# MitchellHansen/voxel-raycaster

Measured on AMD Instinct MI355X. Metric: Mrays/s (primary+shadow), 1920x1080 into depth-12 SVO, higher is better.
Workload: dtype f32

## Files before the change

### __graft_entry__.py

```python
import os
import subprocess
import sys

ROOT = os.path.dirname(os.path.abspath(__file__))
PKG = os.path.join(ROOT, "voxel-raycaster_amd")
CSRC = os.path.join(PKG, "csrc")
HIPCC = os.environ.get("HIPCC", "/opt/rocm/bin/hipcc")
HIP_FLAGS = ["--offload-arch=gfx950", "-O3", "-std=c++17", "-ffp-contract=off", "-fno-slp-vectorize", "-fPIC",
             "-I" + os.path.join(ROOT, "include")]
SOURCES = ["raycast_kernel.hip", "raycast_jump_kernel.hip", "svo_builder_gpu.hip", "empty_boxes.hip", "raycast_query.hip", "box_query.hip", "box_sweep.hip",
           "vrc_api.cpp", "svo_builder.cpp"]
HEADERS = ["vrc_params.h", "raycast_common.hpp", "exact_jump.hpp", "safe_run.hpp", "clcaster.hpp", "shell_scene.hpp", "raycast_query.h",
           "box_query.h", "box_walk.hpp", "box_sweep.h", "vrc_launch.h"]


def _stale(target, deps):
    if not os.path.exists(target):
        return True
    t = os.path.getmtime(target)
    return any(os.path.getmtime(d) > t for d in deps)


def stale() -> bool:
    srcs = [os.path.join(CSRC, s) for s in SOURCES]
    hdrs = [os.path.join(CSRC, h) for h in HEADERS] + [os.path.join(ROOT, "include", "vrc.h")]
    orc = os.path.join(ROOT, "oracle")
    return (_stale(os.path.join(PKG, "libvrc.so"), srcs + hdrs)
            or _stale(os.path.join(orc, "libvrc_oracle.so"), [os.path.join(orc, "vrc_oracle.c"), os.path.join(orc, "vrc_oracle.h")]))
# ... 79 lines not shown
```

### include/vrc.h

```cpp
#ifndef VRC_H
#define VRC_H

#include <stddef.h>
#include <stdint.h>

#ifdef __cplusplus
extern "C" {
#endif

typedef struct vrc_caster vrc_caster;

typedef enum vrc_status {
    VRC_OK = 0,
    VRC_ERR_INVALID_ARGUMENT = 1,
    VRC_ERR_NOT_READY = 2,
    VRC_ERR_DEVICE = 3,
    VRC_ERR_OUT_OF_MEMORY = 4,
    VRC_ERR_NOT_FOUND = 5,
    VRC_ERR_LIMIT = 6
} vrc_status;


int vrc_create(int device_ordinal, vrc_caster **out);
int vrc_destroy(vrc_caster *h);
// ... 134 lines not shown
#define VRC_KERNEL_SVO   1
#define VRC_KERNEL_JUMP  2
#define VRC_KERNEL_ARRAY 3
typedef struct vrc_kernel_info {
    uint32_t struct_size;
    int32_t  family;
    int32_t  n_args;
    int32_t  args[6];
    int32_t  jump_min_run;
    int32_t  lds_rows;
    int32_t  reserved_;
    char     name[96];
} vrc_kernel_info;
int vrc_last_kernel(vrc_caster *h, int32_t rank, vrc_kernel_info *out);

int vrc_get_scheduler_stats(vrc_caster *h, uint64_t out[8]);

int vrc_timing_reset(vrc_caster *h);
int vrc_timing_get(vrc_caster *h, uint64_t *n_launches, double *total_kernel_ms);


int vrc_octree_generate(const int8_t *grid, uint32_t dim, uint64_t buffer_size,
                        int strict_reference, uint64_t **descriptors,
                        uint64_t *n_descriptors, uint64_t *root_index);

int vrc_octree_attachments_from_grid(const int8_t *grid, uint32_t dim, const uint64_t *descriptors,
                                     uint64_t n_descriptors, uint64_t root_index, uint32_t **lookup,
                                     uint64_t **attachments, uint64_t *n_attachments);
int vrc_scene_shell_terrain_attachments(uint32_t depth, uint64_t seed, uint32_t mirror_period,
                                        const uint64_t *descriptors, uint64_t n_descriptors,
// ... 63 lines not shown
```

### voxel-raycaster_amd/__init__.py

```python
from __future__ import annotations

import ctypes as C
import os
from typing import Optional

import numpy as np

_HERE = os.path.dirname(os.path.abspath(__file__))
LIB_PATH = os.environ.get("VRC_LIB_PATH") or os.path.join(_HERE, "libvrc.so")


class VrcError(RuntimeError):
    pass


def _load() -> C.CDLL:
    try:
        import torch
    except ImportError:
        pass
    if not os.path.exists(LIB_PATH):
        raise VrcError(
            f"{LIB_PATH} is missing: build it with `python -c 'import __graft_entry__ as g; g.build()'` "
            "(hipcc --offload-arch=gfx950).  There is no CPU fallback.")
# ... 77 lines not shown
    "vrc_setting_set": (C.c_int, [_H, C.c_char_p, C.c_int64]),
    "vrc_setting_get": (C.c_int, [_H, C.c_char_p, C.POINTER(C.c_int64)]),
    "vrc_validate": (C.c_int, [_H]),
    "vrc_prepare": (C.c_int, [_H]),
    "vrc_compute": (C.c_int, [_H]),
    "vrc_compute_async": (C.c_int, [_H]),
    "vrc_sync": (C.c_int, [_H]),
    "vrc_set_row_tiling": (C.c_int, [_H, C.c_int32, C.c_int32, C.c_int32]),
    "vrc_read_image_f32": (C.c_int, [_H, _f32p, C.c_size_t]),
    "vrc_read_image_rgba8": (C.c_int, [_H, _u8p, C.c_size_t]),
    "vrc_read_hits": (C.c_int, [_H, _i32p, C.c_size_t]),
    "vrc_device_image": (C.c_int, [_H, C.POINTER(C.c_void_p), C.POINTER(C.c_size_t)]),
    "vrc_get_counters": (C.c_int, [_H, C.POINTER(Counters)]),
    "vrc_counters_canonical": (C.c_int, [_H, C.POINTER(C.c_int32)]),
    "vrc_last_kernel": (C.c_int, [_H, C.c_int32, C.POINTER(KernelInfo)]),
    "vrc_get_scheduler_stats": (C.c_int, [_H, _u64p]),
    "vrc_timing_reset": (C.c_int, [_H]),
    "vrc_timing_get": (C.c_int, [_H, _u64p, C.POINTER(C.c_double)]),
    "vrc_octree_generate": (C.c_int, [_i8p, C.c_uint32, C.c_uint64, C.c_int, C.POINTER(_u64p), _u64p, _u64p]),
    "vrc_scene_shell_terrain": (C.c_int, [C.c_uint32, C.c_uint64, C.c_int32, C.c_int, C.POINTER(_u64p), _u64p, _u64p, _i32p]),
    "vrc_octree_attachments_from_grid": (C.c_int, [_i8p, C.c_uint32, _u64p, C.c_uint64, C.c_uint64,
                                                    C.POINTER(C.POINTER(C.c_uint32)), C.POINTER(_u64p), _u64p]),
    "vrc_scene_shell_terrain_attachments": (C.c_int, [C.c_uint32, C.c_uint64, C.c_uint32, _u64p, C.c_uint64, C.c_uint64,
                                                       C.POINTER(C.POINTER(C.c_uint32)), C.POINTER(_u64p), _u64p]),
    "vrc_scene_shell_terrain_dense": (C.c_int, [C.c_uint32, C.c_uint64, C.c_int32, _i8p]),
    "vrc_scene_atlas": (C.c_int, [C.c_int32, C.c_int32, _u8p]),
    "vrc_octree_get_voxel": (C.c_int, [_u64p, C.c_uint64, C.c_uint32, _i32p, _i32p, _i32p, _i32p]),
    "vrc_octree_save": (C.c_int, [C.c_char_p, C.c_uint32, _u64p, C.c_uint64, C.c_uint64, C.POINTER(C.c_uint32), _u64p, C.c_uint64]),
    "vrc_octree_load": (C.c_int, [C.c_char_p, C.POINTER(C.c_uint32), C.POINTER(_u64p), _u64p, _u64p,
                                  C.POINTER(C.POINTER(C.c_uint32)), C.POINTER(_u64p), _u64p]),
# ... 580 lines not shown
    def sweep_boxes_device(self, sweeps_ptr: int, n: int, records_ptr: int, max_events: int = 0, stopping_only: bool = False) -> bool:
        return self._ok(lib.vrc_sweep_boxes_device(self._h, C.c_void_p(sweeps_ptr), int(n), int(max_events),
                                                   SWEEP_STOPPING_ONLY if stopping_only else 0, C.c_void_p(records_ptr)))

    def counters(self) -> dict:
        c = Counters()
        if not self._ok(lib.vrc_get_counters(self._h, C.byref(c))):
            raise VrcError(self.last_error())
        d = c.as_dict()
        canonical = C.c_int32(-1)
        if lib.vrc_counters_canonical(self._h, C.byref(canonical)) != 0:
            raise RuntimeError(self.last_error())
        d["canonical_reads"] = bool(canonical.value)
        return d

    def last_kernel(self, rank: int = 0) -> dict:
        k = KernelInfo()
        k.struct_size = C.sizeof(KernelInfo)
        if not self._ok(lib.vrc_last_kernel(self._h, rank, C.byref(k))):
            raise VrcError(self.last_error())
        return {"family": int(k.family), "args": tuple(int(a) for a in k.args[:k.n_args]), "name": k.name.decode(),
                "jump_min_run": int(k.jump_min_run), "lds_rows": int(k.lds_rows)}

    def scheduler_stats(self) -> dict:
        out = (C.c_uint64 * 8)()
        if not self._ok(lib.vrc_get_scheduler_stats(self._h, out)):
            raise VrcError(self.last_error())
        names = ("wave_step_iterations", "bursts", "event_passes", "event_lanes", "shade_passes", "shade_lanes", "jump_attempts", "jump_successes")
        return {n: int(out[i]) for i, n in enumerate(names)}

# ... 10 lines not shown
```

### voxel-raycaster_amd/csrc/raycast_common.hpp

```cpp
#pragma once

#include <hip/hip_runtime.h>

#include "vrc_params.h"

namespace vrc {

__device__ __forceinline__ float min_cl(float a, float b) { return b < a ? b : a; }
__device__ __forceinline__ float max_cl(float a, float b) { return a < b ? b : a; }
__device__ __forceinline__ float mix_cl(float x, float y, float a) { return x + (y - x) * a; }
__device__ __forceinline__ int isign(float v) { return (v > 0.0f) - (v < 0.0f); }
__device__ __forceinline__ float dot3(float ax, float ay, float az, float bx, float by, float bz) {
    return ax * bx + ay * by + az * bz;
}

struct Vec3 { float x, y, z; };
constexpr unsigned kCountTex = 1u, kCountShadow = 0x100u, kCountBounce = 0x10000u;

__device__ __forceinline__ Vec3 normalize3(Vec3 v) {
    float l2 = dot3(v.x, v.y, v.z, v.x, v.y, v.z);
    if (l2 == 0.0f) return v;
    float l = sqrtf(l2);
    return Vec3{v.x / l, v.y / l, v.z / l};
}
// ... 271 lines not shown
        const int w = blockIdx.x;
        bid = (w / (8 * S)) * 8 + (w & 7);
        sub = (w >> 3) % S;
    }
    return bid < nblocks;
}
template <int kTiles>
__device__ __forceinline__ bool workgroup_exists(const RaycastParams &p) {
    int nblocks, bid, sub;
    return workgroup_group<kTiles>(p, nblocks, bid, sub);
}
template <int kTiles = kTilesPerBlock>
__device__ __forceinline__ bool block_pixel(const RaycastParams &p, int &px, int &py, int &buffer_row) {
    int nblocks, bid, sub;
    if (!workgroup_group<kTiles>(p, nblocks, bid, sub)) return false;
    const int per_xcd = nblocks >> 3;
    int local_ty, bx;
    if (p.xcd_mode == 1 && per_xcd > 0 && bid < (per_xcd << 3) && (p.local_tile_rows & 7) == 0) {
        const int j = bid >> 3;
        local_ty = (j / p.blocks_x) * 8 + (bid & 7);
        bx = j % p.blocks_x;
    } else {
        if (p.xcd_mode == 0 && per_xcd > 0 && bid < (per_xcd << 3)) bid = (bid & 7) * per_xcd + (bid >> 3);
        local_ty = bid / p.blocks_x;
        bx = bid - local_ty * p.blocks_x;
    }
    const int band = local_ty / p.band_tiles;
    const int tile_y = (band * p.tile_world + p.tile_rank) * p.band_tiles + (local_ty - band * p.band_tiles);
    const int wave = sub * kTiles + (threadIdx.x >> 6), lane = threadIdx.x & 63;
    px = (bx * kTilesPerBlock + wave) * kTileW + (lane & (kTileW - 1));
// ... 50 lines not shown
```

### voxel-raycaster_amd/csrc/raycast_kernel.hip

```cpp
#include <hip/hip_runtime.h>

#include <mutex>

#include "exact_jump.hpp"
#include "raycast_common.hpp"
#include "safe_run.hpp"
#include "vrc_launch.h"

#ifndef VRC_RELIGHT_THRESHOLD
#define VRC_RELIGHT_THRESHOLD 64
#endif

namespace vrc {

static_assert(3 * 4 * (int)(sizeof(JumpWord) / sizeof(uint32_t)) == kJumpTableDwordsPerLane, "vrc_api.cpp sizes the global Euclid tables (4 ring rows x 3 pairs x 8 bytes) with kJumpTableDwordsPerLane");

__device__ __forceinline__ uint64_t make_entry(const uint64_t *__restrict__ descriptors, uint64_t index,
                                               uint64_t d) {
    uint64_t base = index + (d & 0x7fffULL);
    if (d & 0x8000ULL) base = descriptors[base];
    return (base << 16) | ((d >> 16) & 0xffffULL);
}

__global__ __launch_bounds__(kBlockThreads) void raycast_array_kernel(const RaycastParams p) {
// ... 45 lines not shown
        ray_finish(r, p, c_desc);
    }
    const unsigned vals[7] = {c_primary, c_shadow, c_desc, c_tex, c_map, c_steps, c_unwritten};
    publish_counters(p, block_ctr, vals, (int)threadIdx.x);
}

#ifndef VRC_MIN_BLOCKS
#define VRC_MIN_BLOCKS (24 / VRC_TILES_PER_BLOCK)
#endif
enum LaneMode { kStep = 0, kEvent = 1, kShade = 2, kDone = 3, kRelight = 4 };

#ifdef VRC_SCHED_STATS
__device__ unsigned long long g_run_hist[3][32];
__device__ unsigned long long g_jump_stats[12];
#endif
#ifdef VRC_TIME_STATS
__device__ unsigned long long g_time_stats[16];
#define VRC_TICK(slot) do { const unsigned long long now_ = __builtin_amdgcn_s_memtime(); if ((tid & 63) == 0) t_acc[slot] += now_ - t_last; t_last = now_; } while (0)
#else
#define VRC_TICK(slot) do { } while (0)
#endif

#ifndef VRC_MIN_BLOCKS_JUMP
#define VRC_MIN_BLOCKS_JUMP (VRC_MIN_BLOCKS - 1)
#endif
constexpr int kHwRegXccId = (3 << 11) | (0 << 6) | 20;
#ifndef VRC_MIN_BLOCKS_JUMP_MULTI
#define VRC_MIN_BLOCKS_JUMP_MULTI VRC_MIN_BLOCKS_JUMP
#endif
constexpr int svo_waves_per_simd(bool jump, bool multi) { return jump ? (multi ? VRC_MIN_BLOCKS_JUMP_MULTI : VRC_MIN_BLOCKS_JUMP) : VRC_MIN_BLOCKS; }
// ... 13 lines not shown
    const int tid = threadIdx.x;
    const int wave_in_block = __builtin_amdgcn_readfirstlane(tid >> 6);
    if (!workgroup_exists<kWgTiles>(p)) {
        if (tid < kCtrCount) p.counters[(long)blockIdx.x * kCtrCount + tid] = 0;
        return;
    }
#ifdef VRC_SCHED_STATS
    constexpr bool kCtrLds = true;
#else
    constexpr bool kCtrLds = kWgTiles > 1;
#endif
    if constexpr (kCtrLds) { if (tid < kCtrCount) block_ctr[tid] = 0; }
#ifdef VRC_TIME_STATS
    __shared__ unsigned long long s_life[3];
    if (tid < 3) s_life[tid] = 0;
#endif
    if (kJump && !kLdsTab && tid == 0) {
        const unsigned per = (unsigned)p.jump_slot_count >> 3;
        const unsigned xcc = (unsigned)__builtin_amdgcn_s_getreg(kHwRegXccId) & 7u;
        const unsigned lo = xcc * per, hi = lo + per;
        unsigned i = lo + (unsigned)(((unsigned long long)(blockIdx.x >> 3) * 2654435761ULL) % per), tries = 0;
        while (atomicCAS(&p.jump_slots[i], 0u, 1u) != 0u) {
            if (++i == hi) i = lo;
            if (++tries >= per) { i = 0xffffffffu; break; }
        }
        s_jump_slot = (int)i;
    }
    __syncthreads();

    int px, py, brow;
// ... 567 lines not shown
    if (l_ok) atomicAdd(&block_ctr[kCtrShadeLanes + 2], (unsigned long long)l_ok);
    if (l_cov) atomicAdd(&block_ctr[kCtrMap], (unsigned long long)l_cov);
#endif
#ifdef VRC_TIME_STATS
    {
        const unsigned long long now_ = __builtin_amdgcn_s_memtime();
        if ((tid_end & 63) == 0) {
            t_acc[8] = now_ - t_begin;
            for (int k = 0; k < 9; k++) atomicAdd(&g_time_stats[k], t_acc[k]);
            atomicAdd(&s_life[0], t_acc[8]);
            atomicMax(&s_life[1], t_acc[8]);
        }
        if (__ballot(c_shadow != 0) != 0 && (tid_end & 63) == 0) atomicOr(&s_life[2], 1ULL);
    }
#endif
    const unsigned vals[7] = {c_primary, c_shadow, c_desc, c_tex, 0u, c_steps, c_unwritten};
    publish_counters<kWgTiles, kCtrLds>(p, block_ctr, vals, tid_end, rounds_left < 0);
    if (kJump && !kLdsTab && tid_end == 0 && s_jump_slot >= 0) atomicExch(&p.jump_slots[s_jump_slot], 0u);
#ifdef VRC_TIME_STATS
    if constexpr (kWgTiles == 1) __syncthreads();
    if (tid_end == 0) {
        const int cls = s_life[2] ? 12 : 9;
        atomicAdd(&g_time_stats[cls], s_life[0]);
        atomicAdd(&g_time_stats[cls + 1], s_life[1] * (unsigned long long)kWgTiles);
        atomicAdd(&g_time_stats[cls + 2], 1ULL);
    }
#endif
}

__global__ void reduce_counters_kernel(const unsigned long long *partials, int nblocks, unsigned long long *out) {
    __shared__ unsigned long long acc[kCtrCount];
    if (threadIdx.x < kCtrCount) acc[threadIdx.x] = 0;
    __syncthreads();
    const int slot = threadIdx.x & (kCtrCount - 1);
    unsigned long long v = 0;
    for (int b = threadIdx.x / kCtrCount; b < nblocks; b += blockDim.x / kCtrCount) v += partials[(long)b * kCtrCount + slot];
    atomicAdd(&acc[slot], v);
    __syncthreads();
    if (threadIdx.x < kCtrCount) out[threadIdx.x] = acc[threadIdx.x];
}

__global__ void frame_setup_kernel(const RaycastParams p) {
    if (threadIdx.x != 0 || blockIdx.x != 0) return;
    int pos[3], corner[3] = {0, 0, 0};
    for (int a = 0; a < 3; a++) pos[a] = (int)floorf(p.cam_pos[a]);
    uint64_t index = p.root_index, d = p.descriptors[index];
    int reads = 1;
    int dimension = 1 << p.log2_dim, res = dimension / 2;
    while (dimension > 1) {
        const int half = dimension / 2;
        int i = 0;
        for (int a = 0; a < 3; a++)
            if (pos[a] >= corner[a] + half) { i |= 1 << a; corner[a] += half; }
        if (!((d >> (16 + i)) & 1ULL)) break;
        if ((d >> (24 + i)) & 1ULL) break;
        dimension = half;
        res /= 2;
        const int before = __popcll((d >> 16) & ((2ULL << i) - 1ULL)) - 1;
        const uint64_t base = (d & 0x8000ULL) ? p.descriptors[index + (d & 0x7fffULL)] : index + (d & 0x7fffULL);
        index = base + (uint64_t)before;
        d = p.descriptors[index];
        reads++;
    }
    for (int a = 0; a < 3; a++) p.frame[a] = p.octree_bias ? (corner[a] - pos[a]) * res / 2 : 0;
    p.frame[3] = reads;
}

__global__ void fill_image_kernel(float4 *image, size_t n) {
    const size_t i = (size_t)blockIdx.x * blockDim.x + threadIdx.x;
    if (i < n) image[i] = make_float4(1.0f, 1.0f, 1.0f, 100.0f / 255.0f);
}

__global__ void pack_rgba8_kernel(const float4 *__restrict__ image, uchar4 *__restrict__ out, size_t n) {
    const size_t i = (size_t)blockIdx.x * blockDim.x + threadIdx.x;
    if (i >= n) return;
    const float4 v = image[i];
    auto q = [](float f) -> unsigned char {
        if (!(f > 0.0f)) f = 0.0f;
        if (f > 1.0f) f = 1.0f;
        return (unsigned char)__float2int_rn(f * 255.0f);
    };
    out[i] = make_uchar4(q(v.x), q(v.y), q(v.z), q(v.w));
}

#ifdef VRC_TIME_STATS
}
extern "C" int vrc_stats_time(unsigned long long *out16, int clear) {
    if (out16 && hipMemcpyFromSymbol(out16, HIP_SYMBOL(vrc::g_time_stats), sizeof(vrc::g_time_stats)) != hipSuccess) return 1;
    if (clear) {
        static unsigned long long zero[16];
        if (hipMemcpyToSymbol(HIP_SYMBOL(vrc::g_time_stats), zero, sizeof(zero)) != hipSuccess) return 1;
    }
    return 0;
}
namespace vrc {
#endif
#ifdef VRC_SCHED_STATS
}
extern "C" int vrc_stats_run_hist(unsigned long long *out96, int clear) {
    if (out96 && hipMemcpyFromSymbol(out96, HIP_SYMBOL(vrc::g_run_hist), sizeof(vrc::g_run_hist)) != hipSuccess) return 1;
    if (out96 && hipMemcpyFromSymbol(out96 + 96, HIP_SYMBOL(vrc::g_jump_stats), sizeof(vrc::g_jump_stats)) != hipSuccess) return 1;
    if (out96 && hipMemcpyFromSymbol(out96 + 108, HIP_SYMBOL(vrc::g_jump_private_solves), sizeof(vrc::g_jump_private_solves)) != hipSuccess) return 1;
    if (clear) {
        static unsigned long long zero[3][32];
        if (hipMemcpyToSymbol(HIP_SYMBOL(vrc::g_run_hist), zero, sizeof(zero)) != hipSuccess) return 1;
        if (hipMemcpyToSymbol(HIP_SYMBOL(vrc::g_jump_stats), zero, sizeof(vrc::g_jump_stats)) != hipSuccess) return 1;
        if (hipMemcpyToSymbol(HIP_SYMBOL(vrc::g_jump_private_solves), zero, sizeof(vrc::g_jump_private_solves)) != hipSuccess) return 1;
    }
    return 0;
}
namespace vrc {
// ... 2 lines not shown
hipError_t launch_fill_image(float *image, size_t n_pixels, hipStream_t stream) {
    (void)hipGetLastError();
    if (!n_pixels) return hipSuccess;
    hipLaunchKernelGGL(fill_image_kernel, dim3((unsigned)((n_pixels + 255) / 256)), dim3(256), 0, stream, reinterpret_cast<float4 *>(image), n_pixels);
    return hipGetLastError();
}

hipError_t launch_pack_rgba8(const float *image, uint8_t *out, size_t n_pixels, hipStream_t stream) {
    (void)hipGetLastError();
    if (!n_pixels) return hipSuccess;
    hipLaunchKernelGGL(pack_rgba8_kernel, dim3((unsigned)((n_pixels + 255) / 256)), dim3(256), 0, stream,
                       reinterpret_cast<const float4 *>(image), reinterpret_cast<uchar4 *>(out), n_pixels);
    return hipGetLastError();
}

hipError_t launch_frame_setup(const RaycastParams &p, hipStream_t stream) {
    (void)hipGetLastError();
    hipLaunchKernelGGL(frame_setup_kernel, dim3(1), dim3(64), 0, stream, p);
    return hipGetLastError();
}

static bool svo_uses_coarse(const RaycastParams &p) {
    return p.coarse != nullptr && p.coarse_log2 >= 1 && p.coarse_log2 <= p.log2_dim - 2;
}
static bool svo_uses_boxes(const RaycastParams &p) { return svo_uses_coarse(p) && p.boxes != nullptr && p.box_aux != nullptr; }
static bool svo_jumps(const RaycastParams &p) { return p.jump_min_run < kJumpOff; }
static int svo_tiles(bool jump, bool multi) { return svo_tiles_per_workgroup(jump, multi); }
static size_t svo_stack_bytes(const RaycastParams &p, int tiles) {
    const int levels = svo_uses_coarse(p) ? p.log2_dim - p.coarse_log2 : (p.log2_dim > 1 ? p.log2_dim - 1 : 1);
    return (size_t)levels * 64 * tiles * (sizeof(uint64_t) + (svo_uses_boxes(p) ? sizeof(uint32_t) : 0)) + (size_t)p.lds_pad_bytes * tiles / kTilesPerBlock;
}
constexpr size_t lds_table_bytes(int rows, int tiles) { return (size_t)(3 * rows) * 64 * tiles * sizeof(JumpWord); }

// ... 104 lines not shown
```

### voxel-raycaster_amd/csrc/vrc_api.cpp

```cpp
#include <hip/hip_runtime.h>

#include <algorithm>
#include <cmath>
#include <cstdarg>
#include <cstdio>
#include <cstring>
#include <initializer_list>
#include <memory>
#include <mutex>
#include <string>
#include <vector>

#include "../../include/vrc.h"
#include "box_query.h"
#include "box_sweep.h"
#include "raycast_query.h"
#include "vrc_launch.h"
#include "vrc_params.h"

namespace {

struct DeviceRestore {
    int dev = -1;
    DeviceRestore() { if (hipGetDevice(&dev) != hipSuccess) { dev = -1; (void)hipGetLastError(); } }
    ~DeviceRestore() { if (dev >= 0) (void)hipSetDevice(dev); }
};

template <class T>
void release(T *&p) {
    if (p) { (void)hipFree(p); p = nullptr; }
// ... 6 lines not shown
struct BoxKey {
    TableKey at; int mode = 0; int64_t levels_asked = 0, records_asked = 0;
    bool operator==(const BoxKey &o) const { return at == o.at && mode == o.mode && levels_asked == o.levels_asked && records_asked == o.records_asked; }
};
template <class Key>
struct Derived {
    Key built, failed;
    bool gave_up = false;
    std::string note;
};

}

struct vrc_setting { std::string name, define; int64_t value; };

struct vrc_tree {
    int device = 0;
    uint64_t *d_desc = nullptr; uint64_t n_desc = 0;
    uint32_t *d_attach_lookup = nullptr; uint64_t *d_attach = nullptr; uint64_t n_attach = 0;
    std::mutex guard;
    uint64_t *d_coarse = nullptr; Derived<TableKey> coarse;
    uint32_t *d_boxes = nullptr, *d_box_aux = nullptr; Derived<BoxKey> boxes; double box_build_seconds = 0.0;
    unsigned long long box_queries_cut = 0;
    int box_levels = 0; uint64_t box_records = 0;
    uint32_t *d_box_child = nullptr; uint64_t *d_box_desc = nullptr, *d_box_pos = nullptr;
    ~vrc_tree() {
        {
            DeviceRestore restore;
            (void)hipSetDevice(device);
            release(d_coarse); release(d_boxes); release(d_box_aux); release(d_box_child); release(d_box_desc); release(d_box_pos);
            release(d_desc); release(d_attach_lookup); release(d_attach);
        }
        (void)hipGetLastError();
// ... 11 lines not shown
    bool own_copy = false;
    int32_t peer_access = -1;
    void *pinned_stage = nullptr; size_t pinned_stage_bytes = 0;
    bool last_frame_boxes = false;
    vrc::LaunchRecord last_launch = {};
    bool last_frame_wrote_hits = false;
    float *d_viewport = nullptr; float *d_image = nullptr; int32_t *d_hits = nullptr; uint8_t *d_rgba8 = nullptr;
    uint32_t *d_jump_cache = nullptr, *d_jump_slots = nullptr; int jump_slot_count = 0, jump_slot_threads = 0;
    int32_t width = 0, height = 0;
    bool sliced = false;
    int32_t buffer_rows = 0;
    uint8_t *d_atlas = nullptr; int32_t atlas_w = 0, atlas_h = 0, tile_w = 0, tile_h = 0;
    unsigned long long *d_partials = nullptr; int partial_blocks = 0;
    unsigned long long *d_counters = nullptr;
    int32_t *d_frame = nullptr;
    unsigned int *wd_flag = nullptr;
    float *d_query_rays = nullptr; int32_t *d_query_out = nullptr; int64_t query_capacity = 0;
    float *d_box_in = nullptr; int32_t *d_box_rec = nullptr; int64_t *d_box_cnt = nullptr; int64_t box_io_capacity = 0;
    int32_t *d_box_vox = nullptr; size_t box_vox_bytes = 0;
    void *d_box_plan = nullptr; int64_t *d_box_scan = nullptr; int32_t *d_box_corner = nullptr; int64_t box_capacity = 0;
    int64_t *d_box_items = nullptr; int64_t box_item_capacity = 0;
    void *d_box_temp = nullptr; size_t box_temp_bytes = 0;
    float *d_sweep_in = nullptr; int32_t *d_sweep_out = nullptr; int64_t sweep_io_capacity = 0;
    int32_t *d_sweep_rec = nullptr, *d_sweep_vox = nullptr; int64_t *d_sweep_cnt = nullptr, *d_sweep_scan = nullptr; int64_t sweep_capacity = 0;
    int64_t sweep_n_big = 0;

    const float *cam_dir = nullptr, *cam_pos = nullptr;
    const float *cam_trig = nullptr;
    const float *lights = nullptr; const int32_t *light_count = nullptr;

// ... 365 lines not shown
    *n = (int32_t)h->peers.size() + 1;
    return VRC_OK;
}

int vrc_destroy(vrc_caster *h) {
    if (!h) return VRC_ERR_INVALID_ARGUMENT;
    for (vrc_caster *q : h->peers) vrc_destroy(q);
    h->peers.clear();
    (void)hipSetDevice(h->device);
    if (h->stream) (void)hipStreamSynchronize(h->stream);
    drain_events(h);
    for (auto &p : h->pool) { (void)hipEventDestroy(p.a); (void)hipEventDestroy(p.b); }
    release_tree(h);
    release(h->d_map);
    release_viewport_buffers(h); release(h->d_atlas);
    release(h->d_partials); release(h->d_counters); release(h->d_frame);
    release_query_staging(h);
    if (h->wd_flag) (void)hipHostFree(h->wd_flag);
    if (h->pinned_stage) (void)hipHostFree(h->pinned_stage);
    if (h->stream) (void)hipStreamDestroy(h->stream);
    delete h;
    return VRC_OK;
}

const char *vrc_last_error(const vrc_caster *h) { return h ? h->error.c_str() : "null handle"; }

int vrc_assign_map(vrc_caster *h, const int8_t *voxels, int32_t dx, int32_t dy, int32_t dz) {
    if (!h || !voxels || dx <= 0 || dy <= 0 || dz <= 0) return fail(h, VRC_ERR_INVALID_ARGUMENT, "assign_map: bad argument");
    HIP_TRY(h, hipSetDevice(h->device));
    release(h->d_map);
    const size_t bytes = (size_t)dx * dy * dz;
// ... 658 lines not shown
    p.blocks_x = (h->width + vrc::kTileW * vrc::kTilesPerBlock - 1) / (vrc::kTileW * vrc::kTilesPerBlock);
    if (svo) derive_from_tree(h, t, p.log2_dim, p.root_index, p.stepping_mode, p);
    p.jump_tables_lds = (int32_t)std::min<int64_t>(2, std::max<int64_t>(0, setting_or(h, "jump_tables_lds", 2)));
    const int lds_rows = vrc::jump_tables_lds_rows(p);
    const bool tables_in_lds = lds_rows > 0;
    p.jump_tables_lds = lds_rows;
    p.jump_min_run = !p.coarse ? vrc::kJumpOff : (int32_t)std::min<int64_t>(vrc::kJumpOff, std::max<int64_t>(1, setting_or(h, "jump_min_run",
                                    p.log2_dim >= (p.boxes ? vrc::kDefaultJumpMinDepthBoxes : vrc::kDefaultJumpMinDepth) ? (tables_in_lds ? vrc::kDefaultJumpMinRunLds : vrc::kDefaultJumpMinRun)
                                                                            : vrc::kJumpOff)));
    p.safe_steps = (int32_t)std::min<int64_t>(256, std::max<int64_t>(2, setting_or(h, "safe_steps",
                                    p.jump_min_run < vrc::kJumpOff ? vrc::kDefaultSafeStepsJump : vrc::kDefaultSafeSteps)));
    const int nblocks = vrc::raycast_workgroups(p), wg_tiles = vrc::raycast_workgroup_tiles(p);
    if (nblocks > h->partial_blocks) {
        release(h->d_partials);
        h->partial_blocks = 0;
        HIP_TRY(h, hipMalloc((void **)&h->d_partials, sizeof(unsigned long long) * vrc::kCtrCount * (size_t)nblocks));
        h->partial_blocks = nblocks;
    }
    p.counters = h->d_partials;
    if (svo && p.stepping_mode == 0 && p.jump_min_run < vrc::kJumpOff && !tables_in_lds) {
        VRC_TRY(ensure_jump_cache(h, nblocks, wg_tiles));
        p.jump_cache = h->d_jump_cache; p.jump_slots = h->d_jump_slots; p.jump_slot_count = h->jump_slot_count;
    }
    h->last_frame_boxes = p.boxes != nullptr;
    h->last_blocks = nblocks;
    h->frames_enqueued++;

    vrc_caster::EvPair ev;
    if (!h->pool.empty()) { ev = h->pool.back(); h->pool.pop_back(); }
    else { HIP_TRY(h, hipEventCreate(&ev.a)); HIP_TRY(h, hipEventCreate(&ev.b)); }

    HIP_TRY(h, vrc::launch_frame_setup(p, h->stream));
    HIP_TRY(h, hipEventRecord(ev.a, h->stream));
    HIP_TRY(h, vrc::launch_raycast(p, h->stream, &h->last_launch));
    HIP_TRY(h, hipEventRecord(ev.b, h->stream));
    h->pending.push_back(ev);
    if (h->pending.size() > 4096) { HIP_TRY(h, hipStreamSynchronize(h->stream)); drain_events(h); }
    return VRC_OK;
}

template <class Enqueue>
int gather_rows(vrc_caster *h, void *host, size_t bpp, Enqueue enqueue) {
    const bool stage = !h->peers.empty() && !host_is_pinned(host, bpp * (size_t)h->width * (size_t)h->height);
    int rc = enqueue(h, stage);
    if (rc != VRC_OK) return rc;
    for (size_t i = 0; i < h->peers.size(); i++) {
        rc = enqueue(h->peers[i], stage);
        if (rc != VRC_OK) return fail(h, rc, "rank %zu: %s", i + 1, h->peers[i]->error.c_str());
    }
    rc = sync_one(h);
// ... 246 lines not shown
    memset(&k, 0, sizeof(k));
    k.family = r.family; k.n_args = r.n_args;
    for (int i = 0; i < 6; i++) k.args[i] = i < r.n_args ? r.args[i] : -1;
    k.jump_min_run = r.jump_min_run; k.lds_rows = r.lds_rows;
    static const char *const family[] = {"", "raycast_svo_kernel", "raycast_jump_kernel", "raycast_array_kernel"};
    std::string name = family[r.family];
    for (int i = 0; i < r.n_args; i++) {
        name += i ? ", " : "<";
        name += ((r.int_args >> i) & 1) ? std::to_string(r.args[i]) : std::string(r.args[i] ? "true" : "false");
    }
    if (r.n_args) name += ">";
    snprintf(k.name, sizeof(k.name), "%s", name.c_str());
    const uint32_t n = std::min<uint32_t>(out->struct_size, (uint32_t)sizeof(k));
    k.struct_size = n;
    memcpy(out, &k, n);
    return VRC_OK;
}

int vrc_get_scheduler_stats(vrc_caster *h, uint64_t out[8]) {
    if (!h || !out) return VRC_ERR_INVALID_ARGUMENT;
    vrc_counters tmp;
    int rc = vrc_get_counters(h, &tmp);
    if (rc != VRC_OK) return rc;
    for (int i = 0; i < 8; i++) out[i] = h->sched_stats[i];
    return VRC_OK;
}

int vrc_timing_reset(vrc_caster *h) {
    if (!h) return VRC_ERR_INVALID_ARGUMENT;
    int rc = vrc_sync(h);
// ... 340 lines not shown
```

### voxel-raycaster_amd/csrc/vrc_launch.h

```cpp
#pragma once

#include <hip/hip_runtime.h>

#include <stdint.h>

#include <string>

#include "../../include/vrc.h"

namespace vrc {

struct RaycastParams;
struct LaunchRecord;
struct QueryParams;
struct BoxParams;
struct SweepParams;

hipError_t launch_fill_image(float *image, size_t n_pixels, hipStream_t stream);
hipError_t launch_pack_rgba8(const float *image, uint8_t *out, size_t n_pixels, hipStream_t stream);
hipError_t launch_frame_setup(const RaycastParams &p, hipStream_t stream);
int jump_tables_lds_rows(const RaycastParams &p);
int raycast_workgroup_tiles(const RaycastParams &p);
int raycast_workgroups(const RaycastParams &p);
hipError_t launch_raycast(const RaycastParams &p, hipStream_t stream, LaunchRecord *rec);
hipError_t launch_reduce_counters(const unsigned long long *partials, int nblocks, unsigned long long *out,
                                  hipStream_t stream);

hipError_t launch_raycast_jump(const RaycastParams &p, hipStream_t stream, LaunchRecord *rec);
hipError_t launch_coarse_build(const uint64_t *descriptors, uint64_t root_index, int log2_dim, int lc, uint64_t *out, hipStream_t stream);

hipError_t launch_box_positions(const uint64_t *descriptors, uint64_t n_desc, uint64_t root_index, int n, uint64_t *pos, hipStream_t stream);
hipError_t launch_box_build(const uint64_t *descriptors, uint64_t n_desc, uint64_t root_index, int n, int lc, uint64_t *pos_tmp,
                            uint32_t *boxes, uint32_t *aux, hipStream_t stream);
struct BoxUpper { uint64_t *desc = nullptr, *pos = nullptr; uint32_t *child = nullptr, *boxes = nullptr; uint64_t count = 0; int levels = 0; };
hipError_t launch_box_build_upper(const uint64_t *descriptors, uint64_t root_index, int n, int lc, uint64_t max_records, int max_levels,
// ... 30 lines not shown
```

### voxel-raycaster_amd/csrc/vrc_params.h

```cpp
#pragma once

#include <stdint.h>

namespace vrc {

#ifndef VRC_TILE_W
#define VRC_TILE_W 8
#endif
constexpr int kTileW = VRC_TILE_W;
constexpr int kTileH = 64 / VRC_TILE_W;
static_assert((kTileW & (kTileW - 1)) == 0 && kTileW >= 1 && kTileW <= 64, "tile width must be a power of two <= 64");
#ifndef VRC_TILES_PER_BLOCK
#define VRC_TILES_PER_BLOCK 4
#endif
constexpr int kTilesPerBlock = VRC_TILES_PER_BLOCK;
constexpr int kBlockThreads = 64 * kTilesPerBlock;
#ifndef VRC_SVO_TILES
#define VRC_SVO_TILES 1
#endif
constexpr int svo_tiles_per_workgroup(bool , bool ) { return VRC_SVO_TILES; }
static_assert(VRC_SVO_TILES >= 1 && VRC_TILES_PER_BLOCK % VRC_SVO_TILES == 0, "a workgroup is a whole fraction of a block");
constexpr int svo_workgroups(int groups, int tiles) {
    return tiles == kTilesPerBlock ? groups : ((groups + 7) / 8) * 8 * (kTilesPerBlock / tiles);
}
// ... 97 lines not shown
    int32_t lds_pad_bytes;
    int32_t xcd_mode;
    int32_t tile_rank, tile_world, band_tiles;
    int32_t blocks_x;
    int32_t local_tile_rows;
    int32_t row_sliced;
    int32_t stepping_mode;
    const uint64_t *coarse;
    int32_t coarse_log2;
    const uint32_t *boxes;
    const uint32_t *box_aux;
    const uint32_t *box_child;
    int32_t box_levels;
    unsigned long long *counters;
    unsigned int *watchdog_flag;
};

}
```

Baseline: 2576.

## Add cost-based workgroup launch ordering and skip redundant frame setup

Adds an optional launch-order permutation. The frame setup kernel uses per-workgroup step counters from the previous frame to rank runs of tile groups. With automatic mode, expensive groups are dispatched first to reduce tail imbalance; reversed and shuffled modes are also offered. Separately, the frame setup kernel is skipped when the tree, root, bias and camera position are unchanged, which saves one small launch per repeated frame. The reordering is off by default (launch_order=0), so by default only the setup skip runs. That skip relies on the cache key catching every change to the scene.

Result: no change. 2589, median of 6 (+0.5%).

```diff
diff --git a/__graft_entry__.py b/__graft_entry__.py
--- a/__graft_entry__.py
+++ b/__graft_entry__.py
@@ -11,7 +11,7 @@
 SOURCES = ["raycast_kernel.hip", "raycast_jump_kernel.hip", "svo_builder_gpu.hip", "empty_boxes.hip", "raycast_query.hip", "box_query.hip", "box_sweep.hip",
            "vrc_api.cpp", "svo_builder.cpp"]
 HEADERS = ["vrc_params.h", "raycast_common.hpp", "exact_jump.hpp", "safe_run.hpp", "clcaster.hpp", "shell_scene.hpp", "raycast_query.h",
-           "box_query.h", "box_walk.hpp", "box_sweep.h", "vrc_launch.h"]
+           "box_query.h", "box_walk.hpp", "box_sweep.h", "vrc_launch.h", "launch_order.hpp"]
 
 
 def _stale(target, deps):
diff --git a/include/vrc.h b/include/vrc.h
--- a/include/vrc.h
+++ b/include/vrc.h
@@ -172,6 +172,8 @@
 } vrc_kernel_info;
 int vrc_last_kernel(vrc_caster *h, int32_t rank, vrc_kernel_info *out);
 
+int vrc_read_launch_order(vrc_caster *h, int32_t rank, uint32_t *out, int32_t capacity, int32_t *count);
+
 int vrc_get_scheduler_stats(vrc_caster *h, uint64_t out[8]);
 
 int vrc_timing_reset(vrc_caster *h);
diff --git a/voxel-raycaster_amd/__init__.py b/voxel-raycaster_amd/__init__.py
--- a/voxel-raycaster_amd/__init__.py
+++ b/voxel-raycaster_amd/__init__.py
@@ -115,6 +115,7 @@
     "vrc_get_counters": (C.c_int, [_H, C.POINTER(Counters)]),
     "vrc_counters_canonical": (C.c_int, [_H, C.POINTER(C.c_int32)]),
     "vrc_last_kernel": (C.c_int, [_H, C.c_int32, C.POINTER(KernelInfo)]),
+    "vrc_read_launch_order": (C.c_int, [_H, C.c_int32, C.POINTER(C.c_uint32), C.c_int32, _i32p]),
     "vrc_get_scheduler_stats": (C.c_int, [_H, _u64p]),
     "vrc_timing_reset": (C.c_int, [_H]),
     "vrc_timing_get": (C.c_int, [_H, _u64p, C.POINTER(C.c_double)]),
@@ -725,6 +726,15 @@
         d["canonical_reads"] = bool(canonical.value)
         return d
 
+    def launch_order(self, rank: int = 0) -> np.ndarray:
+        n = C.c_int32(0)
+        if not self._ok(lib.vrc_read_launch_order(self._h, rank, None, 0, C.byref(n))):
+            raise VrcError(self.last_error())
+        out = np.empty(n.value, dtype=np.uint32)
+        if n.value and not self._ok(lib.vrc_read_launch_order(self._h, rank, out.ctypes.data_as(C.POINTER(C.c_uint32)), n.value, C.byref(n))):
+            raise VrcError(self.last_error())
+        return out
+
     def last_kernel(self, rank: int = 0) -> dict:
         k = KernelInfo()
         k.struct_size = C.sizeof(KernelInfo)
diff --git a/voxel-raycaster_amd/csrc/launch_order.hpp b/voxel-raycaster_amd/csrc/launch_order.hpp
--- /dev/null
+++ b/voxel-raycaster_amd/csrc/launch_order.hpp
@@ -0,0 +1,112 @@
+#pragma once
+
+#include <stdint.h>
+
+#if defined(__HIPCC__)
+#define VRC_LO __host__ __device__ __forceinline__
+#else
+#define VRC_LO inline
+#endif
+
+namespace vrc {
+
+constexpr int kLaunchRunGroups = 8;
+enum LaunchOrderMode { kLaunchOrderOff = 0, kLaunchOrderAuto = 1, kLaunchOrderReversed = 2, kLaunchOrderShuffled = 3 };
+#ifndef VRC_DEFAULT_LAUNCH_ORDER
+#define VRC_DEFAULT_LAUNCH_ORDER 0
+#endif
+#ifndef VRC_DEFAULT_LAUNCH_FRONT
+#define VRC_DEFAULT_LAUNCH_FRONT 50
+#endif
+#ifndef VRC_DEFAULT_LAUNCH_BACK
+#define VRC_DEFAULT_LAUNCH_BACK 0
+#endif
+#ifndef VRC_DEFAULT_LAUNCH_COST
+#define VRC_DEFAULT_LAUNCH_COST 5
+#endif
+constexpr int kDefaultLaunchCost = VRC_DEFAULT_LAUNCH_COST;
+constexpr int kDefaultLaunchOrder = VRC_DEFAULT_LAUNCH_ORDER, kDefaultLaunchFront = VRC_DEFAULT_LAUNCH_FRONT, kDefaultLaunchBack = VRC_DEFAULT_LAUNCH_BACK;
+
+struct LaunchOrderShape {
+    int groups;
+    int slots;
+    int runs;
+};
+VRC_LO LaunchOrderShape launch_order_shape(int groups) {
+    LaunchOrderShape s;
+    s.groups = groups < 0 ? 0 : groups;
+    const int per_xcd = (s.groups + 7) / 8;
+    s.slots = per_xcd * 8;
+    s.runs = (per_xcd + kLaunchRunGroups - 1) / kLaunchRunGroups;
+    return s;
+}
+VRC_LO int launch_order_scratch_words(const LaunchOrderShape &s) { return s.slots + 16 * s.runs; }
+VRC_LO int launch_list_groups(const LaunchOrderShape &s, int k) { return s.groups > k ? (s.groups - k + 7) / 8 : 0; }
+VRC_LO int launch_run_groups(const LaunchOrderShape &s, int k, int r) {
+    const int left = launch_list_groups(s, k) - r * kLaunchRunGroups;
+    return left <= 0 ? 0 : (left < kLaunchRunGroups ? left : kLaunchRunGroups);
+}
+VRC_LO uint32_t launch_order_hash(uint32_t x) {
+    x ^= x >> 16; x *= 0x7feb352du; x ^= x >> 15; x *= 0x846ca68bu; x ^= x >> 16;
+    return x;
+}
+
+VRC_LO void launch_order_run_costs(const LaunchOrderShape &s, const uint32_t *group_cost, uint32_t *run_cost, int tid, int nth) {
+    for (int f = tid; f < 8 * s.runs; f += nth) {
+        const int k = f & 7, r = f >> 3, len = launch_run_groups(s, k, r);
+        uint32_t c = 0;
+        for (int i = 0; i < len; i++) c += group_cost[(r * kLaunchRunGroups + i) * 8 + k];
+        run_cost[f] = c;
+    }
+}
+VRC_LO void launch_order_run_keys(const LaunchOrderShape &s, int mode, uint32_t seed, int front_permille, int back_permille,
+                                  const uint32_t *run_cost, uint32_t *run_key, int tid, int nth) {
+    const int R = s.runs;
+    const int n_front = (int)((long long)R * front_permille / 1000), n_back = (int)((long long)R * back_permille / 1000);
+    for (int f = tid; f < 8 * R; f += nth) {
+        const int k = f & 7, r = f >> 3;
+        uint32_t key = (uint32_t)r;
+        if (mode == kLaunchOrderReversed) key = (uint32_t)(R - 1 - r);
+        else if (mode == kLaunchOrderShuffled) key = launch_order_hash(((uint32_t)r * 8u + (uint32_t)k) ^ launch_order_hash(seed));
+        else if (mode == kLaunchOrderAuto) {
+            const uint32_t mine = run_cost[f];
+            int rank = 0;
+            for (int q = 0; q < R; q++) {
+                const uint32_t c = run_cost[q * 8 + k];
+                rank += (c > mine || (c == mine && q < r)) ? 1 : 0;
+            }
+            key = rank < n_front ? 0u : (rank >= R - n_back ? 2u : 1u);
+        }
+        run_key[f] = key;
+    }
+}
+VRC_LO void launch_order_write(const LaunchOrderShape &s, const uint32_t *run_key, uint32_t *order, int tid, int nth) {
+    const int R = s.runs;
+    for (int f = tid; f < 8 * R; f += nth) {
+        const int k = f & 7, r = f >> 3, len = launch_run_groups(s, k, r);
+        if (len == 0) continue;
+        const uint32_t mine = run_key[f];
+        int at = 0;
+        for (int q = 0; q < R; q++) {
+            const uint32_t c = run_key[q * 8 + k];
+            if (c < mine || (c == mine && q < r)) at += launch_run_groups(s, k, q);
+        }
+        for (int i = 0; i < len; i++) order[(at + i) * 8 + k] = (uint32_t)((r * kLaunchRunGroups + i) * 8 + k);
+    }
+    for (int g = s.groups + tid; g < s.slots; g += nth) order[g] = (uint32_t)g;
+}
+VRC_LO void launch_order_identity(const LaunchOrderShape &s, uint32_t *order, int tid, int nth) {
+    for (int g = tid; g < s.slots; g += nth) order[g] = (uint32_t)g;
+}
+
+inline void launch_order_build(int groups, int mode, uint32_t seed, int front_permille, int back_permille, const uint32_t *group_cost,
+                               uint32_t *order, uint32_t *scratch) {
+    const LaunchOrderShape s = launch_order_shape(groups);
+    uint32_t *run_cost = scratch + s.slots, *run_key = run_cost + 8 * s.runs;
+    if (mode == kLaunchOrderOff) { launch_order_identity(s, order, 0, 1); return; }
+    launch_order_run_costs(s, group_cost, run_cost, 0, 1);
+    launch_order_run_keys(s, mode, seed, front_permille, back_permille, run_cost, run_key, 0, 1);
+    launch_order_write(s, run_key, order, 0, 1);
+}
+
+}
diff --git a/voxel-raycaster_amd/csrc/raycast_common.hpp b/voxel-raycaster_amd/csrc/raycast_common.hpp
--- a/voxel-raycaster_amd/csrc/raycast_common.hpp
+++ b/voxel-raycaster_amd/csrc/raycast_common.hpp
@@ -309,6 +309,7 @@
 __device__ __forceinline__ bool block_pixel(const RaycastParams &p, int &px, int &py, int &buffer_row) {
     int nblocks, bid, sub;
     if (!workgroup_group<kTiles>(p, nblocks, bid, sub)) return false;
+    if constexpr (kTiles < kTilesPerBlock) { if (p.group_order) bid = (int)p.group_order[bid]; }
     const int per_xcd = nblocks >> 3;
     int local_ty, bx;
     if (p.xcd_mode == 1 && per_xcd > 0 && bid < (per_xcd << 3) && (p.local_tile_rows & 7) == 0) {
diff --git a/voxel-raycaster_amd/csrc/raycast_kernel.hip b/voxel-raycaster_amd/csrc/raycast_kernel.hip
--- a/voxel-raycaster_amd/csrc/raycast_kernel.hip
+++ b/voxel-raycaster_amd/csrc/raycast_kernel.hip
@@ -3,6 +3,7 @@
 #include <mutex>
 
 #include "exact_jump.hpp"
+#include "launch_order.hpp"
 #include "raycast_common.hpp"
 #include "safe_run.hpp"
 #include "vrc_launch.h"
@@ -83,6 +84,15 @@
 __device__ unsigned long long g_run_hist[3][32];
 __device__ unsigned long long g_jump_stats[12];
 #endif
+#if defined(VRC_TIME_STATS) && !defined(VRC_TIMELINE)
+#define VRC_TIMELINE
+#endif
+#ifdef VRC_TIMELINE
+__device__ unsigned long long *g_timeline;
+__device__ unsigned int g_timeline_cap;
+constexpr int kTimelineWords = 8;
+constexpr int kHwRegHwId = (31 << 11) | (0 << 6) | 4;
+#endif
 #ifdef VRC_TIME_STATS
 __device__ unsigned long long g_time_stats[16];
 #define VRC_TICK(slot) do { const unsigned long long now_ = __builtin_amdgcn_s_memtime(); if ((tid & 63) == 0) t_acc[slot] += now_ - t_last; t_last = now_; } while (0)
@@ -126,6 +136,15 @@
 #ifdef VRC_TIME_STATS
     __shared__ unsigned long long s_life[3];
     if (tid < 3) s_life[tid] = 0;
+#endif
+#ifdef VRC_TIMELINE
+    if (tid == 0) {
+        unsigned long long *tl = g_timeline;
+        if (tl && blockIdx.x < g_timeline_cap) {
+            tl[kTimelineWords * (size_t)blockIdx.x] = __builtin_amdgcn_s_memtime();
+            tl[kTimelineWords * (size_t)blockIdx.x + 2] = __builtin_amdgcn_s_memrealtime();
+        }
+    }
 #endif
     if (kJump && !kLdsTab && tid == 0) {
         const unsigned per = (unsigned)p.jump_slot_count >> 3;
@@ -723,6 +742,9 @@
         if (__ballot(c_shadow != 0) != 0 && (tid_end & 63) == 0) atomicOr(&s_life[2], 1ULL);
     }
 #endif
+#ifdef VRC_TIMELINE
+    const bool tl_shadow = __ballot(c_shadow != 0) != 0;
+#endif
     const unsigned vals[7] = {c_primary, c_shadow, c_desc, c_tex, 0u, c_steps, c_unwritten};
     publish_counters<kWgTiles, kCtrLds>(p, block_ctr, vals, tid_end, rounds_left < 0);
     if (kJump && !kLdsTab && tid_end == 0 && s_jump_slot >= 0) atomicExch(&p.jump_slots[s_jump_slot], 0u);
@@ -735,6 +757,18 @@
         atomicAdd(&g_time_stats[cls + 2], 1ULL);
     }
 #endif
+#ifdef VRC_TIMELINE
+    if (tid_end == 0) {
+        unsigned long long *tl = g_timeline;
+        if (tl && blockIdx.x < g_timeline_cap) {
+            const unsigned long long xcc = (unsigned long long)((unsigned)__builtin_amdgcn_s_getreg(kHwRegXccId) & 15u);
+            unsigned long long *rec = tl + kTimelineWords * (size_t)blockIdx.x;
+            rec[1] = __builtin_amdgcn_s_memtime(); rec[3] = __builtin_amdgcn_s_memrealtime();
+            rec[4] = (unsigned long long)blockIdx.x | (xcc << 32) | ((tl_shadow ? 1ULL : 0ULL) << 40) | (1ULL << 63);
+            rec[5] = (unsigned long long)(unsigned)__builtin_amdgcn_s_getreg(kHwRegHwId);
+        }
+    }
+#endif
 }
 
 __global__ void reduce_counters_kernel(const unsigned long long *partials, int nblocks, unsigned long long *out) {
@@ -749,8 +783,7 @@
     if (threadIdx.x < kCtrCount) out[threadIdx.x] = acc[threadIdx.x];
 }
 
-__global__ void frame_setup_kernel(const RaycastParams p) {
-    if (threadIdx.x != 0 || blockIdx.x != 0) return;
+__device__ void frame_bias(const RaycastParams &p) {
     int pos[3], corner[3] = {0, 0, 0};
     for (int a = 0; a < 3; a++) pos[a] = (int)floorf(p.cam_pos[a]);
     uint64_t index = p.root_index, d = p.descriptors[index];
@@ -775,6 +808,50 @@
     p.frame[3] = reads;
 }
 
+__global__ __launch_bounds__(1024) void frame_setup_kernel(const RaycastParams p, const FrameOrderJob job) {
+    const int tid = (int)threadIdx.x, nth = (int)blockDim.x;
+    if (!job.order) {
+        if (tid == 0) frame_bias(p);
+        return;
+    }
+    __shared__ int s_bad;
+    const LaunchOrderShape sh = launch_order_shape(job.groups);
+    constexpr int kLdsRuns = 512;
+    __shared__ uint32_t s_run[2 * 8 * kLdsRuns];
+    uint32_t *group_cost = job.scratch;
+    uint32_t *run_cost = sh.runs <= kLdsRuns ? s_run : group_cost + sh.slots, *run_key = run_cost + 8 * sh.runs;
+    const bool gather = job.mode == kLaunchOrderAuto && job.history != 0;
+    if (tid == 0) s_bad = 0;
+    __syncthreads();
+    if (tid == nth - 1) {
+        frame_bias(p);
+    } else if (gather) {
+        const int S = job.wg_per_group;
+        for (int s = tid; s < sh.slots; s += nth - 1) {
+            const int j = s >> 3, k = s & 7;
+            unsigned long long steps = 0, marked = 0;
+            for (int sub = 0; sub < S; sub++) {
+                const unsigned long long *row = p.counters + (long)(8 * (S * j + sub) + k) * kCtrCount;
+                steps += row[job.cost_column];
+                marked |= row[kCtrWatchdog];
+            }
+            const uint32_t g = job.order[s];
+            if (marked || g >= (uint32_t)sh.slots) s_bad = 1;
+            else group_cost[g] = (uint32_t)(steps >> 4 < (1ULL << 24) ? steps >> 4 : (1ULL << 24));
+        }
+    }
+    __syncthreads();
+    if (job.mode == kLaunchOrderOff || (job.mode == kLaunchOrderAuto && (!gather || s_bad))) {
+        launch_order_identity(sh, job.order, tid, nth);
+        return;
+    }
+    launch_order_run_costs(sh, group_cost, run_cost, tid, nth);
+    __syncthreads();
+    launch_order_run_keys(sh, job.mode, job.seed, job.front_permille, job.back_permille, run_cost, run_key, tid, nth);
+    __syncthreads();
+    launch_order_write(sh, run_key, job.order, tid, nth);
+}
+
 __global__ void fill_image_kernel(float4 *image, size_t n) {
     const size_t i = (size_t)blockIdx.x * blockDim.x + threadIdx.x;
     if (i < n) image[i] = make_float4(1.0f, 1.0f, 1.0f, 100.0f / 255.0f);
@@ -804,6 +881,16 @@
 }
 namespace vrc {
 #endif
+#ifdef VRC_TIMELINE
+}
+extern "C" int vrc_stats_timeline(unsigned long long *device_records, unsigned int records) {
+    if (hipDeviceSynchronize() != hipSuccess) return 1;
+    if (hipMemcpyToSymbol(HIP_SYMBOL(vrc::g_timeline_cap), &records, sizeof(records)) != hipSuccess) return 1;
+    if (hipMemcpyToSymbol(HIP_SYMBOL(vrc::g_timeline), &device_records, sizeof(device_records)) != hipSuccess) return 1;
+    return 0;
+}
+namespace vrc {
+#endif
 #ifdef VRC_SCHED_STATS
 }
 extern "C" int vrc_stats_run_hist(unsigned long long *out96, int clear) {
@@ -836,9 +923,9 @@
     return hipGetLastError();
 }
 
-hipError_t launch_frame_setup(const RaycastParams &p, hipStream_t stream) {
+hipError_t launch_frame_setup(const RaycastParams &p, const FrameOrderJob &job, hipStream_t stream) {
     (void)hipGetLastError();
-    hipLaunchKernelGGL(frame_setup_kernel, dim3(1), dim3(64), 0, stream, p);
+    hipLaunchKernelGGL(frame_setup_kernel, dim3(1), dim3(job.order ? 1024 : 64), 0, stream, p, job);
     return hipGetLastError();
 }
 
diff --git a/voxel-raycaster_amd/csrc/vrc_api.cpp b/voxel-raycaster_amd/csrc/vrc_api.cpp
--- a/voxel-raycaster_amd/csrc/vrc_api.cpp
+++ b/voxel-raycaster_amd/csrc/vrc_api.cpp
@@ -1,6 +1,7 @@
 #include <hip/hip_runtime.h>
 
 #include <algorithm>
+#include <atomic>
 #include <cmath>
 #include <cstdarg>
 #include <cstdio>
@@ -14,6 +15,7 @@
 #include "../../include/vrc.h"
 #include "box_query.h"
 #include "box_sweep.h"
+#include "launch_order.hpp"
 #include "raycast_query.h"
 #include "vrc_launch.h"
 #include "vrc_params.h"
@@ -50,9 +52,15 @@
 
 struct vrc_setting { std::string name, define; int64_t value; };
 
+static uint64_t next_tree_serial() {
+    static std::atomic<uint64_t> next{1};
+    return next.fetch_add(1);
+}
+
 struct vrc_tree {
     int device = 0;
     uint64_t *d_desc = nullptr; uint64_t n_desc = 0;
+    uint64_t serial = next_tree_serial();
     uint32_t *d_attach_lookup = nullptr; uint64_t *d_attach = nullptr; uint64_t n_attach = 0;
     std::mutex guard;
     uint64_t *d_coarse = nullptr; Derived<TableKey> coarse;
@@ -94,6 +102,23 @@
     unsigned long long *d_partials = nullptr; int partial_blocks = 0;
     unsigned long long *d_counters = nullptr;
     int32_t *d_frame = nullptr;
+    struct FrameKey {
+        bool valid = false; uint64_t tree = 0, root = 0; int32_t log2_dim = 0, octree_bias = 0; float cam_pos[3] = {0, 0, 0};
+        bool operator==(const FrameKey &o) const {
+            return valid == o.valid && tree == o.tree && root == o.root && log2_dim == o.log2_dim && octree_bias == o.octree_bias &&
+                   memcmp(cam_pos, o.cam_pos, sizeof(cam_pos)) == 0;
+        }
+    } frame_key;
+    uint32_t *d_order = nullptr; int order_slots = 0;
+    struct OrderKey {
+        bool valid = false; int32_t width = 0, height = 0, rank = 0, world = 0, band = 0, sliced = 0, workgroups = 0, groups = 0, blocks_x = 0, wg_tiles = 0;
+        int32_t instance[6] = {0, 0, 0, 0, 0, 0};
+        bool operator==(const OrderKey &o) const {
+            return valid == o.valid && width == o.width && height == o.height && rank == o.rank && world == o.world && band == o.band &&
+                   sliced == o.sliced && workgroups == o.workgroups && groups == o.groups && blocks_x == o.blocks_x && wg_tiles == o.wg_tiles &&
+                   memcmp(instance, o.instance, sizeof(instance)) == 0;
+        }
+    } order_key;
     unsigned int *wd_flag = nullptr;
     float *d_query_rays = nullptr; int32_t *d_query_out = nullptr; int64_t query_capacity = 0;
     float *d_box_in = nullptr; int32_t *d_box_rec = nullptr; int64_t *d_box_cnt = nullptr; int64_t box_io_capacity = 0;
@@ -489,7 +514,7 @@
     release_tree(h);
     release(h->d_map);
     release_viewport_buffers(h); release(h->d_atlas);
-    release(h->d_partials); release(h->d_counters); release(h->d_frame);
+    release(h->d_partials); release(h->d_counters); release(h->d_frame); release(h->d_order);
     release_query_staging(h);
     if (h->wd_flag) (void)hipHostFree(h->wd_flag);
     if (h->pinned_stage) (void)hipHostFree(h->pinned_stage);
@@ -1178,6 +1203,7 @@
     if (nblocks > h->partial_blocks) {
         release(h->d_partials);
         h->partial_blocks = 0;
+        h->order_key.valid = false;
         HIP_TRY(h, hipMalloc((void **)&h->d_partials, sizeof(unsigned long long) * vrc::kCtrCount * (size_t)nblocks));
         h->partial_blocks = nblocks;
     }
@@ -1186,6 +1212,38 @@
         VRC_TRY(ensure_jump_cache(h, nblocks, wg_tiles));
         p.jump_cache = h->d_jump_cache; p.jump_slots = h->d_jump_slots; p.jump_slot_count = h->jump_slot_count;
     }
+    vrc::FrameOrderJob job;
+    memset(&job, 0, sizeof(job));
+    vrc_caster::OrderKey order_key;
+    const int64_t order_mode = setting_or(h, "launch_order", vrc::kDefaultLaunchOrder);
+    if (order_mode < 0 || order_mode > vrc::kLaunchOrderShuffled)
+        return fail(h, VRC_ERR_INVALID_ARGUMENT, "compute: launch_order must be 0 (off), 1 (automatic), 2 (reversed) or 3 (shuffled)");
+    if (order_mode != vrc::kLaunchOrderOff && svo && p.stepping_mode == 0 && wg_tiles < vrc::kTilesPerBlock && p.blocks_x * p.local_tile_rows > 0) {
+        const vrc::LaunchOrderShape shape = vrc::launch_order_shape(p.blocks_x * p.local_tile_rows);
+        if (shape.slots > h->order_slots) {
+            release(h->d_order);
+            h->order_slots = 0;
+            h->order_key.valid = false;
+            HIP_TRY(h, hipMalloc((void **)&h->d_order, sizeof(uint32_t) * ((size_t)shape.slots + (size_t)vrc::launch_order_scratch_words(shape))));
+            h->order_slots = shape.slots;
+        }
+        job.order = h->d_order; job.scratch = h->d_order + h->order_slots;
+        job.groups = shape.groups; job.wg_per_group = vrc::kTilesPerBlock / wg_tiles;
+        job.mode = (int32_t)order_mode; job.seed = (uint32_t)setting_or(h, "launch_order_seed", 1);
+        job.front_permille = (int32_t)std::min<int64_t>(1000, std::max<int64_t>(0, setting_or(h, "launch_order_front", vrc::kDefaultLaunchFront)));
+        job.back_permille = (int32_t)std::min<int64_t>(1000 - job.front_permille, std::max<int64_t>(0, setting_or(h, "launch_order_back", vrc::kDefaultLaunchBack)));
+        job.cost_column = (int32_t)std::min<int64_t>(vrc::kCtrUnwritten, std::max<int64_t>(vrc::kCtrPrimary, setting_or(h, "launch_order_cost", vrc::kDefaultLaunchCost)));
+        order_key.valid = true; order_key.width = h->width; order_key.height = h->height; order_key.rank = h->tile_rank; order_key.world = h->tile_world;
+        order_key.band = h->band_rows; order_key.sliced = h->sliced ? 1 : 0; order_key.workgroups = nblocks; order_key.groups = shape.groups;
+        order_key.blocks_x = p.blocks_x; order_key.wg_tiles = wg_tiles;
+        const int32_t instance[6] = {p.log2_dim, p.jump_min_run, p.jump_tables_lds, p.light_count, p.coarse ? p.coarse_log2 : -1, p.boxes ? 1 : 0};
+        memcpy(order_key.instance, instance, sizeof(instance));
+        job.history = (h->order_key.valid && order_key == h->order_key) ? 1 : 0;
+        p.group_order = h->d_order;
+    }
+    vrc_caster::FrameKey frame_key;
+    frame_key.valid = true; frame_key.tree = t->serial; frame_key.root = p.root_index; frame_key.log2_dim = p.log2_dim; frame_key.octree_bias = p.octree_bias;
+    for (int a = 0; a < 3; a++) frame_key.cam_pos[a] = p.cam_pos[a];
     h->last_frame_boxes = p.boxes != nullptr;
     h->last_blocks = nblocks;
     h->frames_enqueued++;
@@ -1194,10 +1252,16 @@
     if (!h->pool.empty()) { ev = h->pool.back(); h->pool.pop_back(); }
     else { HIP_TRY(h, hipEventCreate(&ev.a)); HIP_TRY(h, hipEventCreate(&ev.b)); }
 
-    HIP_TRY(h, vrc::launch_frame_setup(p, h->stream));
+    if (job.order || !(frame_key == h->frame_key)) {
+        h->frame_key.valid = false;
+        HIP_TRY(h, vrc::launch_frame_setup(p, job, h->stream));
+        h->frame_key = frame_key;
+    }
     HIP_TRY(h, hipEventRecord(ev.a, h->stream));
+    h->order_key.valid = false;
     HIP_TRY(h, vrc::launch_raycast(p, h->stream, &h->last_launch));
     HIP_TRY(h, hipEventRecord(ev.b, h->stream));
+    if (job.order) h->order_key = order_key;
     h->pending.push_back(ev);
     if (h->pending.size() > 4096) { HIP_TRY(h, hipStreamSynchronize(h->stream)); drain_events(h); }
     return VRC_OK;
@@ -1474,6 +1538,20 @@
     const uint32_t n = std::min<uint32_t>(out->struct_size, (uint32_t)sizeof(k));
     k.struct_size = n;
     memcpy(out, &k, n);
+    return VRC_OK;
+}
+
+int vrc_read_launch_order(vrc_caster *h, int32_t rank, uint32_t *out, int32_t capacity, int32_t *count) {
+    if (!h || !count || capacity < 0 || (capacity > 0 && !out) || rank < 0 || rank > (int32_t)h->peers.size()) return VRC_ERR_INVALID_ARGUMENT;
+    vrc_caster *q = rank == 0 ? h : h->peers[rank - 1];
+    *count = (q->order_key.valid && q->d_order) ? vrc::launch_order_shape(q->order_key.groups).slots : 0;
+    const int32_t n = std::min(*count, capacity);
+    if (n > 0) {
+        HIP_TRY(h, hipSetDevice(q->device));
+        HIP_TRY(h, hipMemcpyAsync(out, q->d_order, sizeof(uint32_t) * (size_t)n, hipMemcpyDeviceToHost, q->stream));
+        HIP_TRY(h, hipStreamSynchronize(q->stream));
+        if (rank != 0) HIP_TRY(h, hipSetDevice(h->device));
+    }
     return VRC_OK;
 }
 
diff --git a/voxel-raycaster_amd/csrc/vrc_launch.h b/voxel-raycaster_amd/csrc/vrc_launch.h
--- a/voxel-raycaster_amd/csrc/vrc_launch.h
+++ b/voxel-raycaster_amd/csrc/vrc_launch.h
@@ -12,13 +12,14 @@
 
 struct RaycastParams;
 struct LaunchRecord;
+struct FrameOrderJob;
 struct QueryParams;
 struct BoxParams;
 struct SweepParams;
 
 hipError_t launch_fill_image(float *image, size_t n_pixels, hipStream_t stream);
 hipError_t launch_pack_rgba8(const float *image, uint8_t *out, size_t n_pixels, hipStream_t stream);
-hipError_t launch_frame_setup(const RaycastParams &p, hipStream_t stream);
+hipError_t launch_frame_setup(const RaycastParams &p, const FrameOrderJob &job, hipStream_t stream);
 int jump_tables_lds_rows(const RaycastParams &p);
 int raycast_workgroup_tiles(const RaycastParams &p);
 int raycast_workgroups(const RaycastParams &p);
diff --git a/voxel-raycaster_amd/csrc/vrc_params.h b/voxel-raycaster_amd/csrc/vrc_params.h
--- a/voxel-raycaster_amd/csrc/vrc_params.h
+++ b/voxel-raycaster_amd/csrc/vrc_params.h
@@ -135,6 +135,19 @@
     int32_t box_levels;
     unsigned long long *counters;
     unsigned int *watchdog_flag;
+    const uint32_t *group_order;
+};
+
+struct FrameOrderJob {
+    uint32_t *order;
+    uint32_t *scratch;
+    int32_t groups;
+    int32_t wg_per_group;
+    int32_t mode;
+    uint32_t seed;
+    int32_t front_permille, back_permille;
+    int32_t cost_column;
+    int32_t history;
 };
 
 }
```
